# AdamClixby/Modulate

Hardware: NVIDIA B200
Metric: ark_dtb_decrypt_throughput (higher is better)
Workload: dtype u8

## Files before the change

### modulate_b200/csrc/cycle_kernels.cu

```cuda
#include "cycle_kernels.cuh"
#include "lcg.h"

#include <cstdlib>

namespace modk {

using modlcg::mulmod;
using modlcg::step_lazy;
using modlcg::low8_canonical;

#ifndef MODK_CANON_FMA_MASK
#define MODK_CANON_FMA_MASK 0x5
#endif
#ifndef MODK_MIN_CTAS
#define MODK_MIN_CTAS 10
#endif
#ifndef MODK_MIN_CTAS_INLINE
#define MODK_MIN_CTAS_INLINE 8
#endif
#ifndef MODK_MIN_CTAS_COAL
#define MODK_MIN_CTAS_COAL 10
#endif
#ifndef MODK_STAGE
#define MODK_STAGE 1
#endif
#ifndef MODK_EDGE_ROUNDS
#define MODK_EDGE_ROUNDS 1
#endif
#ifndef MODK_STAGE_SEQ
#define MODK_STAGE_SEQ 1
#endif
#ifndef MODK_GENERAL_FULL
#define MODK_GENERAL_FULL 1
#endif
#ifndef MODK_HOIST_POW
#define MODK_HOIST_POW 1
#endif
#ifndef MODK_REC_PREFETCH
#define MODK_REC_PREFETCH 2048
#endif

constexpr int kTw0Size = 1024;
constexpr int kTw1Size = (int)(((1ull << 32) / kTileBytes) / kTw0Size + 2);

__constant__ uint32_t c_tw0[kTw0Size];
__constant__ uint32_t c_tw1[kTw1Size];
__constant__ uint32_t c_ainv[16];
__device__ uint32_t g_chunk_pow2[kChunksPerTile];

__device__ __forceinline__ uint32_t jump_lazy(uint32_t st, uint32_t y2)
{
    const uint64_t p = (uint64_t)st * (uint64_t)y2;
    return (uint32_t)(p >> 32) + ((uint32_t)p >> 1);
}


__device__ __forceinline__ uint4 ldg128(uint64_t addr)
{
    uint4 r;
    asm volatile("ld.global.v4.u32 {%0, %1, %2, %3}, [%4];" : "=r"(r.x), "=r"(r.y), "=r"(r.z), "=r"(r.w) : "l"(addr));
    return r;
}

__device__ __forceinline__ void stg128(uint64_t addr, const uint4& v)
{
    asm volatile("st.global.v4.u32 [%0], {%1, %2, %3, %4};" ::"l"(addr), "r"(v.x), "r"(v.y), "r"(v.z), "r"(v.w));
}

#if MODK_STAGE

__device__ __forceinline__ uint32_t smem_u32(const void* p) { return (uint32_t)__cvta_generic_to_shared(p); }

__device__ __forceinline__ void mbar_init(uint32_t bar, uint32_t count)
{
    asm volatile("mbarrier.init.shared::cta.b64 [%0], %1;" ::"r"(bar), "r"(count));
    asm volatile("fence.mbarrier_init.release.cluster;" ::: "memory");
}

__device__ __forceinline__ void mbar_expect_tx(uint32_t bar, uint32_t bytes)
{
    asm volatile("mbarrier.arrive.expect_tx.shared::cta.b64 _, [%0], %1;" ::"r"(bar), "r"(bytes) : "memory");
}

__device__ __forceinline__ void mbar_wait(uint32_t bar, uint32_t parity)
{
    asm volatile(
        "{\n"
        ".reg .pred p;\n"
        "MODK_WAIT:\n"
        "mbarrier.try_wait.parity.shared::cta.b64 p, [%0], %1;\n"
        "@p bra MODK_DONE;\n"
        "bra MODK_WAIT;\n"
        "MODK_DONE:\n"
        "}\n" ::"r"(bar), "r"(parity) : "memory");
}

__device__ __forceinline__ void bulk_g2s(uint32_t dst_smem, uint64_t src_gmem, uint32_t bytes, uint32_t bar)
{
    asm volatile("cp.async.bulk.shared::cluster.global.mbarrier::complete_tx::bytes [%0], [%1], %2, [%3];" ::"r"(dst_smem),
                 "l"(src_gmem), "r"(bytes), "r"(bar)
                 : "memory");
}

__device__ __forceinline__ uint4 lds128(uint32_t addr)
{
    uint4 r;
    asm volatile("ld.shared.v4.u32 {%0, %1, %2, %3}, [%4];" : "=r"(r.x), "=r"(r.y), "=r"(r.z), "=r"(r.w) : "r"(addr));
    return r;
}
#endif


__device__ __forceinline__ uint32_t low8_canonical_fma(uint32_t s, uint32_t two)
{
    uint32_t r;
    asm("mad.hi.u32 %0, %1, %2, %1;" : "=r"(r) : "r"(s), "r"(two));
    return r;
}

// ... 231 lines not shown
        return;
    }
    constexpr bool kStaged = MODK_STAGE != 0;
#if MODK_STAGE
    if (threadIdx.x == 0) {
        const uint32_t bytes = 16u * (n_valid + (shift ? 1u : 0u));
        mbar_expect_tx(bar, bytes);
        bulk_g2s(stage, src_tile, bytes, bar);
    }
#endif
#if MODK_GENERAL_FULL
    if (geom == kFullGeom) {
        switch (shift ? (int)(shift >> 2) : -1) {
        case -1: process_tile<-1, U, kStaged, true>(src_tile, dst_tile, st, n_valid, head, tail, bs, idx0, pw, a.two, stage, bar); break;
        case 0: process_tile<0, U, kStaged, true>(src_tile, dst_tile, st, n_valid, head, tail, bs, idx0, pw, a.two, stage, bar); break;
        case 1: process_tile<1, U, kStaged, true>(src_tile, dst_tile, st, n_valid, head, tail, bs, idx0, pw, a.two, stage, bar); break;
        case 2: process_tile<2, U, kStaged, true>(src_tile, dst_tile, st, n_valid, head, tail, bs, idx0, pw, a.two, stage, bar); break;
        default: process_tile<3, U, kStaged, true>(src_tile, dst_tile, st, n_valid, head, tail, bs, idx0, pw, a.two, stage, bar); break;
        }
        return;
    }
#endif
    if (shift == 0u) {
        process_tile<-1, U, kStaged>(src_tile, dst_tile, st, n_valid, head, tail, bs, idx0, pw, a.two, stage, bar);
    } else {
        switch (shift >> 2) {
        case 0: process_tile<0, U, kStaged>(src_tile, dst_tile, st, n_valid, head, tail, bs, idx0, pw, a.two, stage, bar); break;
        case 1: process_tile<1, U, kStaged>(src_tile, dst_tile, st, n_valid, head, tail, bs, idx0, pw, a.two, stage, bar); break;
        case 2: process_tile<2, U, kStaged>(src_tile, dst_tile, st, n_valid, head, tail, bs, idx0, pw, a.two, stage, bar); break;
        default: process_tile<3, U, kStaged>(src_tile, dst_tile, st, n_valid, head, tail, bs, idx0, pw, a.two, stage, bar); break;
        }
    }
}

__device__ __forceinline__ uint32_t tile_start_state(uint32_t n0, uint32_t h0, uint32_t tin)
{
    const uint32_t st = mulmod(n0, c_ainv[h0]);
    return mulmod(st, mulmod(c_tw0[tin & (uint32_t)(kTw0Size - 1)], c_tw1[tin / (uint32_t)kTw0Size]));
}

__device__ __forceinline__ TileRec make_tile_rec(uint64_t src_off, uint64_t dst_off, uint32_t len, uint32_t n0,
                                                 uint32_t tin, uint32_t dst_align, uint32_t entry)
{
    const uint32_t h0 = (dst_align + (uint32_t)dst_off) & 15u;
    const uint64_t span = (uint64_t)h0 + len;
    const uint32_t nchunks = (uint32_t)((span + 15u) >> 4);
    const uint32_t c_begin = tin * (uint32_t)kChunksPerTile;
    const uint32_t n_valid = min((uint32_t)kChunksPerTile, nchunks - c_begin);
    const bool last = c_begin + n_valid == nchunks;
    TileRec r;
    r.src_rel = (int64_t)src_off - (int64_t)h0 + 16ll * (int64_t)c_begin;
    r.dst_rel = (int64_t)dst_off - (int64_t)h0 + 16ll * (int64_t)c_begin;
    r.state = tile_start_state(n0, h0, tin);
    r.geom = pack_geom(n_valid, tin == 0u ? h0 : 0u, last ? (((uint32_t)span - 1u) & 15u) + 1u : 16u);
    r.entry = entry;
    r.pad = 0u;
    return r;
}

#if MODK_STAGE
#define MODK_STAGE_SETUP                                                                          \
    uint32_t stage = 0u, bar = 0u;                                                                \
    if (kGeneral) {                                                                               \
        __shared__ __align__(128) uint8_t s_stage[kTileBytes + 16];                               \
        __shared__ __align__(8) uint64_t s_bar;                                                   \
        stage = smem_u32(s_stage);                                                                \
        bar = smem_u32(&s_bar);                                                                   \
        if (threadIdx.x == 0)                                                                     \
            mbar_init(bar, 1u);                                                                   \
        __syncthreads();                                                                          \
    }
#else
#define MODK_STAGE_SETUP const uint32_t stage = 0u, bar = 0u;
#endif

template <int U>
__device__ __forceinline__ void load_chunk_pows(uint32_t (&pw)[U], uint32_t idx0)
{
#pragma unroll
    for (int u = 0; u < U; ++u)
        pw[u] = __ldg(&g_chunk_pow2[idx0 + (uint32_t)u * (uint32_t)kThreadsPerCta]);
}

template <bool kGeneral>
__global__ void __launch_bounds__(kThreadsPerCta, kGeneral ? MODK_MIN_CTAS : MODK_MIN_CTAS_COAL)
cycle_batch_kernel(const BatchArgs a)
{
    MODK_STAGE_SETUP
    const uint4* p = reinterpret_cast<const uint4*>(a.tiles + blockIdx.x);
    uint32_t pw[kUnroll];
#if MODK_HOIST_POW
    load_chunk_pows<kUnroll>(pw, threadIdx.x);
#endif
    const uint4 lo = __ldg(p);
    const uint4 hi = __ldg(p + 1);
#if MODK_REC_PREFETCH
    if (threadIdx.x == 0 && a.n_tiles - blockIdx.x > (uint32_t)MODK_REC_PREFETCH) {
        const uint64_t ahead = (uint64_t)(a.tiles + blockIdx.x + MODK_REC_PREFETCH);
        if ((ahead & 127u) == 0u)
            asm volatile("prefetch.global.L2 [%0];" ::"l"(ahead));
    }
#endif
    const int64_t src_rel = (int64_t)((uint64_t)lo.x | ((uint64_t)lo.y << 32));
    const int64_t dst_rel = (int64_t)((uint64_t)lo.z | ((uint64_t)lo.w << 32));
#if !MODK_HOIST_POW
    load_chunk_pows<kUnroll>(pw, threadIdx.x);
#endif
    run_tile<kUnroll, kGeneral>(a, src_rel, dst_rel, hi.x, hi.y, threadIdx.x, pw, stage, bar);
}

template <bool kGeneral>
__global__ void __launch_bounds__(kThreadsPerCta, kGeneral ? MODK_MIN_CTAS_INLINE : MODK_MIN_CTAS_COAL)
cycle_inline_kernel(const BatchArgs a, const __grid_constant__ InlineDescs in)
{
    MODK_STAGE_SETUP
    uint32_t pw[kUnroll];
    load_chunk_pows<kUnroll>(pw, threadIdx.x);
    const uint32_t tile = blockIdx.x;
    const uint32_t e = tile / a.tiles_per_entry;
    const DevDesc& d = in.d[e];
    const TileRec r = make_tile_rec(d.src_off, d.dst_off, d.len, d.neg_state, tile - d.first_tile,
                                    (uint32_t)(uintptr_t)a.dst & 15u, e);
    run_tile<kUnroll, kGeneral>(a, r.src_rel, r.dst_rel, r.state, r.geom, threadIdx.x, pw, stage, bar);
}

__global__ void build_tiles_kernel(const DevDesc* __restrict__ descs, uint32_t n_descs, uint32_t dst_align,
                                   TileRec* __restrict__ tiles, uint32_t n_tiles)
{
    const uint32_t t = blockIdx.x * blockDim.x + threadIdx.x;
    if (t >= n_tiles)
        return;
    uint32_t lo = 0, hi = n_descs;
    while (hi - lo > 1) {
        const uint32_t mid = lo + ((hi - lo) >> 1);
        if (descs[mid].first_tile <= t)
            lo = mid;
        else
            hi = mid;
    }
    const DevDesc d = descs[lo];
    tiles[t] = make_tile_rec(d.src_off, d.dst_off, d.len, d.neg_state, t - d.first_tile, dst_align, lo);
}


cudaError_t upload_tables()
{
    static uint32_t h_tw0[kTw0Size], h_tw1[kTw1Size], h_ainv[16], h_chunk[kChunksPerTile];
    static const bool built = []() {
        for (int j = 0; j < kTw0Size; ++j)
            h_tw0[j] = modlcg::pow_a((uint64_t)kTileBytes * (uint64_t)j);
        for (int j = 0; j < kTw1Size; ++j)
            h_tw1[j] = modlcg::pow_a((uint64_t)kTileBytes * (uint64_t)kTw0Size * (uint64_t)j);
        for (int h = 0; h < 16; ++h)
            h_ainv[h] = modlcg::pow_a_inv((uint64_t)h);
        for (int j = 0; j < kChunksPerTile; ++j)
            h_chunk[j] = 2u * modlcg::pow_a(16ull * (uint64_t)j);
        return true;
    }();
    (void)built;
    cudaError_t err;
    if ((err = cudaMemcpyToSymbol(c_tw0, h_tw0, sizeof(h_tw0))) != cudaSuccess) return err;
    if ((err = cudaMemcpyToSymbol(c_tw1, h_tw1, sizeof(h_tw1))) != cudaSuccess) return err;
    if ((err = cudaMemcpyToSymbol(c_ainv, h_ainv, sizeof(h_ainv))) != cudaSuccess) return err;
    if ((err = cudaMemcpyToSymbol(g_chunk_pow2, h_chunk, sizeof(h_chunk))) != cudaSuccess) return err;
    return cudaSuccess;
}

constexpr uint32_t kMaxGrid = 0x7FFFFFFFu;

static bool coaligned(const BatchArgs& a)
{
    if (a.uniform_delta < 0 || getenv("MOD_FORCE_GENERAL") != nullptr)
        return false;
    return (((uintptr_t)a.src - (uintptr_t)a.dst + (uintptr_t)a.uniform_delta) & 15u) == 0u;
}

cudaError_t launch_batch(const BatchArgs& args, cudaStream_t stream)
{
    for (uint32_t t0 = 0; t0 < args.n_tiles;) {
        const uint32_t n = args.n_tiles - t0 < kMaxGrid ? args.n_tiles - t0 : kMaxGrid;
        BatchArgs a = args;
        a.tiles = args.tiles + t0;
        a.n_tiles = n;
        if (coaligned(args))
            cycle_batch_kernel<false><<<n, kThreadsPerCta, 0, stream>>>(a);
        else
            cycle_batch_kernel<true><<<n, kThreadsPerCta, 0, stream>>>(a);
        const cudaError_t err = cudaGetLastError();
        if (err != cudaSuccess)
            return err;
        t0 += n;
    }
    return cudaSuccess;
}

cudaError_t launch_batch_inline(const BatchArgs& args, const InlineDescs& descs, cudaStream_t stream)
{
    if (args.n_tiles == 0)
        return cudaSuccess;
    if (coaligned(args))
        cycle_inline_kernel<false><<<args.n_tiles, kThreadsPerCta, 0, stream>>>(args, descs);
    else
        cycle_inline_kernel<true><<<args.n_tiles, kThreadsPerCta, 0, stream>>>(args, descs);
    return cudaGetLastError();
}

cudaError_t launch_build_tiles(const DevDesc* descs, uint32_t n_descs, uint32_t dst_align, TileRec* tiles,
                               uint32_t n_tiles, cudaStream_t stream)
{
    if (n_tiles == 0)
        return cudaSuccess;
    const unsigned threads = 256;
    build_tiles_kernel<<<(n_tiles + threads - 1) / threads, threads, 0, stream>>>(descs, n_descs, dst_align,
                                                                                 tiles, n_tiles);
    return cudaGetLastError();
}

}
```

### modulate_b200/csrc/cycle_kernels.cuh

```cuda
#pragma once

#include <cuda_runtime.h>
#include <stdint.h>

namespace modk {

#ifndef MODK_THREADS
#define MODK_THREADS 128
#endif
#ifndef MODK_UNROLL
#define MODK_UNROLL 4
#endif
constexpr int kThreadsPerCta = MODK_THREADS;
constexpr int kUnroll = MODK_UNROLL;
constexpr int kChunksPerTile = kThreadsPerCta * kUnroll;
constexpr uint32_t kTileBytes = 16u * kChunksPerTile;
constexpr int kMaxInlineDescs = 64;
static_assert(kChunksPerTile <= 2048, "TileRec::geom holds the chunk count in 12 bits");

struct __align__(16) DevDesc {
    uint64_t src_off;
    uint64_t dst_off;
    uint32_t len;
    int32_t key;
    uint32_t first_tile;
    uint32_t neg_state;
};

struct __align__(16) TileRec {
    int64_t src_rel;
    int64_t dst_rel;
    uint32_t state;
    uint32_t geom;
    uint32_t entry;
    uint32_t pad;
};

__host__ __device__ inline uint32_t pack_geom(uint32_t n_valid, uint32_t head, uint32_t tail)
{
    return n_valid | (head << 12) | (tail << 16);
}

struct InlineDescs {
    DevDesc d[kMaxInlineDescs];
};

struct BatchArgs {
    const uint8_t* src;
    uint8_t* dst;
    const TileRec* tiles;
    uint32_t n_tiles;
    uint32_t tiles_per_entry;
    uint64_t src_lo16;
    uint64_t src_hi16;
    uint32_t two = 2;
    int32_t uniform_delta = -1;
};

__host__ __device__ inline uint32_t tiles_for_entry(uint32_t h0, uint32_t len)
{
    if (len == 0)
        return 0;
    const uint64_t chunks = ((uint64_t)h0 + len + 15u) >> 4;
    return (uint32_t)((chunks + (uint32_t)kChunksPerTile - 1) / (uint32_t)kChunksPerTile);
}

cudaError_t upload_tables();
cudaError_t launch_batch(const BatchArgs& args, cudaStream_t stream);
cudaError_t launch_batch_inline(const BatchArgs& args, const InlineDescs& descs, cudaStream_t stream);
cudaError_t launch_build_tiles(const DevDesc* descs, uint32_t n_descs, uint32_t dst_align, TileRec* tiles,
                               uint32_t n_tiles, cudaStream_t stream);

}
```

### modulate_b200/csrc/mod_abi.cu

```cuda
#include "../../include/modulate_b200.h"

#include <cuda_runtime.h>

#include <algorithm>
#include <atomic>
#include <chrono>
#include <cstdarg>
#include <cstdio>
#include <cstdlib>
#include <cstring>
#include <exception>
#include <mutex>
#include <new>
#include <string>
#include <thread>
#include <vector>

#include "batch_cut.h"
#include "cycle_kernels.cuh"
#include "lcg.h"

namespace {

#ifndef MOD_PIPE_SLOTS
// ... 232 lines not shown
        return fail(MOD_ERR_NOMEM, "cudaHostAlloc(%llu) failed: %s", (unsigned long long)need, cudaGetErrorString(e));
    }
    *have = need;
    return MOD_OK;
}

cudaError_t pool_alloc(DeviceCtx& c, uint64_t bytes, void** out, uint64_t* got)
{
    bytes = std::max<uint64_t>(256, (bytes + 255) & ~255ull);
    {
        std::lock_guard<std::mutex> lock(c.pool_mu);
        size_t best = c.pool.size();
        for (size_t i = 0; i < c.pool.size(); ++i)
            if (c.pool[i].bytes >= bytes && c.pool[i].bytes / 4 <= bytes && (best == c.pool.size() || c.pool[i].bytes < c.pool[best].bytes))
                best = i;
        if (best != c.pool.size()) {
            *out = c.pool[best].p;
            *got = c.pool[best].bytes;
            c.pool.erase(c.pool.begin() + (long)best);
            return cudaSuccess;
        }
    }
    *got = bytes;
    return cudaMalloc(out, bytes);
}

void pool_free(DeviceCtx& c, void* p, uint64_t bytes)
{
    if (!p)
        return;
    if (bytes <= kPoolMaxBlockBytes && c.ready.load(std::memory_order_acquire)) {
        std::lock_guard<std::mutex> lock(c.pool_mu);
        if (c.pool.size() >= kPoolBlocks) {
            size_t smallest = 0;
            for (size_t i = 1; i < c.pool.size(); ++i)
                if (c.pool[i].bytes < c.pool[smallest].bytes)
                    smallest = i;
            if (c.pool[smallest].bytes < bytes) {
                cudaFree(c.pool[smallest].p);
                c.pool[smallest] = DeviceCtx::Block{p, bytes};
                return;
            }
        } else {
            c.pool.push_back(DeviceCtx::Block{p, bytes});
            return;
        }
    }
    cudaFree(p);
}

int launch_contiguous(const uint8_t* d_src, uint8_t* d_dst, uint64_t len, int32_t key, cudaStream_t stream)
{
    if (len == 0)
        return MOD_OK;
    const uint32_t h0 = (uint32_t)((uintptr_t)d_dst & 15u);
    const uint64_t piece = kMaxPiece;
    const uint64_t src_lo16 = ((uint64_t)(uintptr_t)d_src + 15u) & ~15ull;
    const uint64_t src_hi16 = ((uint64_t)(uintptr_t)d_src + len) & ~15ull;
    const uint32_t tpe = modk::tiles_for_entry(h0, (uint32_t)piece);
    uint64_t done = 0;
    const uint32_t k0 = modlcg::key_residue(key);
    while (done < len) {
        modk::InlineDescs in;
        modk::BatchArgs args;
        uint32_t n = 0, tiles = 0;
        const uint64_t group_base = done;
        while (done < len && n < (uint32_t)modk::kMaxInlineDescs) {
            const uint64_t this_len = std::min(piece, len - done);
            modk::DevDesc& d = in.d[n];
            d.src_off = done - group_base;
            d.dst_off = done - group_base;
            d.len = (uint32_t)this_len;
            d.key = (int32_t)modlcg::mulmod(k0, modlcg::pow_a(done));
            d.first_tile = n * tpe;
            d.neg_state = modlcg::key_to_neg_state(d.key);
            tiles = n * tpe + modk::tiles_for_entry(h0, (uint32_t)this_len);
            done += this_len;
            ++n;
        }
        args.src = d_src + group_base;
        args.dst = d_dst + group_base;
        args.tiles = nullptr;
        args.n_tiles = tiles;
        args.tiles_per_entry = tpe;
        args.src_lo16 = src_lo16;
        args.src_hi16 = src_hi16;
        args.uniform_delta = 0;
        CUDA_TRY(modk::launch_batch_inline(args, in, stream));
        g_launches.fetch_add(1, std::memory_order_relaxed);
    }
    return MOD_OK;
}

int cycle_host(DeviceCtx& c, uint8_t* host, uint64_t len, int32_t key)
{
    std::lock_guard<std::mutex> lock(c.mu);
    uint64_t slice = env_u64("MOD_SLICE_BYTES", 16ull << 20);
    slice = std::max<uint64_t>(4096, slice & ~4095ull);
    if (len < slice * 2)
        slice = std::max<uint64_t>(4096, ((len / kPipeSlots) + 4095) & ~4095ull);
    const int slots = (int)std::min<uint64_t>(kPipeSlots, (len + slice - 1) / slice);
    for (int i = 0; i < slots; ++i) {
        const int rc = grow(&c.slice_buf[i], &c.slice_bytes[i], slice);
        if (rc != MOD_OK)
            return rc;
    }
    const uint32_t k0 = modlcg::key_residue(key);
    int rc = MOD_OK;
    cudaError_t e = cudaSuccess;
    uint64_t pos = 0;
    const uint64_t head = len >= 4 * slice ? ((kCopyAlign - ((uintptr_t)host & (kCopyAlign - 1))) & (kCopyAlign - 1)) : 0;
    for (uint64_t i = 0; pos < len && rc == MOD_OK && e == cudaSuccess; ++i) {
        const int slot = (int)(i % kPipeSlots);
        const uint64_t n = i == 0 && head ? head : std::min(slice, len - pos);
        cudaStream_t s = c.pipe_stream[slot];
        uint8_t* d = (uint8_t*)c.slice_buf[slot];
        e = cudaMemcpyAsync(d, host + pos, n, cudaMemcpyHostToDevice, s);
        if (e != cudaSuccess)
            break;
        rc = launch_contiguous(d, d, n, (int32_t)modlcg::mulmod(k0, modlcg::pow_a(pos)), s);
        if (rc != MOD_OK)
            break;
        e = cudaMemcpyAsync(host + pos, d, n, cudaMemcpyDeviceToHost, s);
        pos += n;
    }
    const cudaError_t ed = drain(c);
    if (rc != MOD_OK)
        return rc;
    if (e == cudaSuccess)
        e = ed;
    if (e != cudaSuccess)
        return fail(MOD_ERR_CUDA, "mod_cycle: %s", cudaGetErrorString(e));
    return MOD_OK;
}

int validate_descs(const char* who, const mod_desc* descs, uint64_t n, uint64_t src_bytes, uint64_t dst_bytes)
{
    for (uint64_t i = 0; i < n; ++i) {
        const mod_desc& d = descs[i];
        if (d.src_off > src_bytes || (uint64_t)d.len > src_bytes - d.src_off)
            return fail(MOD_ERR_ARG, "%s: descriptor %llu: source range [%llu, +%u) leaves the %llu-byte buffer", who,
                        (unsigned long long)i, (unsigned long long)d.src_off, d.len, (unsigned long long)src_bytes);
        if (d.dst_off > dst_bytes || (uint64_t)d.len > dst_bytes - d.dst_off)
            return fail(MOD_ERR_ARG, "%s: descriptor %llu: destination range [%llu, +%u) leaves the %llu-byte buffer", who,
                        (unsigned long long)i, (unsigned long long)d.dst_off, d.len, (unsigned long long)dst_bytes);
    }
    return MOD_OK;
}

int32_t uniform_delta_of(const mod_desc* descs, uint64_t n)
{
    int32_t delta = -1;
    for (uint64_t i = 0; i < n; ++i) {
        if (!descs[i].len)
            continue;
        const int32_t d = (int32_t)((descs[i].src_off - descs[i].dst_off) & 15u);
        if (delta < 0)
            delta = d;
        else if (delta != d)
            return -1;
    }
    return delta;
}

int expand_descs(const mod_desc* descs, uint64_t n, uint32_t dst_align, modk::DevDesc* out, uint64_t* tiles_out,
                 uint64_t* payload_out)
{
    uint64_t tiles = 0, payload = 0;
    for (uint64_t i = 0; i < n; ++i) {
        const mod_desc& d = descs[i];
        modk::DevDesc& o = out[i];
// ... 153 lines not shown
                    gaps.push_back(gap);
                }
                runs.back().second = b1;
            } else {
                runs.emplace_back(b0, b1);
            }
            prev_rank = rank[idx];
        }
    };
    std::vector<std::pair<uint64_t, uint64_t>> runs;
    bool holes = false;
    for (const Group& g : groups) {
        merged_runs(g, runs, false);
        if (runs.size() > 64) {
            holes = true;
            break;
        }
    }
    if (holes)
        whole();

    const bool split_downloads = env_u64("MOD_SPLIT_DOWNLOADS", 1) != 0;
    const int slots = (int)std::min<size_t>(kPipeSlots, groups.size());
    {
        uint64_t s_need = 0, d_need = 0;
        for (const Group& g : groups) {
            s_need = std::max<uint64_t>(s_need, (g.s_lo & 15u) + (g.s_hi - g.s_lo) + 3 * kCopyAlign);
            d_need = std::max<uint64_t>(d_need, g.d_hi - (g.d_lo & ~15ull) + kCopyAlign);
        }
        for (int k = 0; k < slots; ++k) {
            if ((rc = grow(&c.slot_src[k], &c.slot_src_bytes[k], s_need)) != MOD_OK)
                return rc;
            if ((rc = grow(&c.slot_dst[k], &c.slot_dst_bytes[k], d_need)) != MOD_OK)
                return rc;
        }
    }

    cudaError_t e = cudaMemcpyAsync(c.ws_descs, c.h_descs, n * sizeof(modk::DevDesc), cudaMemcpyHostToDevice, c.pipe_stream[0]);
    if (e == cudaSuccess) {
        e = modk::launch_build_tiles((const modk::DevDesc*)c.ws_descs, (uint32_t)n, 0, (modk::TileRec*)c.ws_tiles,
                                     (uint32_t)plan_tiles, c.pipe_stream[0]);
        g_launches.fetch_add(1, std::memory_order_relaxed);
    }
    if (e == cudaSuccess)
        e = cudaEventRecord(c.plan_ready, c.pipe_stream[0]);
    const modk::TileRec* d_tiles = (const modk::TileRec*)c.ws_tiles;
    const int32_t uniform_delta = uniform_delta_of(descs, n);
    const double t_plan = now_ms();

    const uint64_t fail_group = env_u64("MOD_TEST_FAIL_GROUP", UINT64_MAX);
    for (size_t gi = 0; gi < groups.size() && e == cudaSuccess; ++gi) {
        if (gi == fail_group) {
            e = cudaErrorUnknown;
            break;
        }
        const Group& g = groups[gi];
        const int k = (int)(gi % (size_t)slots);
        cudaStream_t s = c.pipe_stream[k];
        const uint64_t d_lo16 = g.d_lo & ~15ull;
        uint64_t up_lo = g.s_lo, up_hi = g.s_hi;
        uint8_t* win_src = (uint8_t*)c.slot_src[k] + (g.s_lo & 15u);
        uint8_t* win_dst = (uint8_t*)c.slot_dst[k];
        if (align_copies) {
            up_lo -= std::min<uint64_t>(g.s_lo, (uintptr_t)(src + g.s_lo) & (kCopyAlign - 1));
            up_hi = std::min<uint64_t>(src_bytes, g.s_hi + ((kCopyAlign - ((uintptr_t)(src + g.s_hi) & (kCopyAlign - 1))) & (kCopyAlign - 1)));
            win_src = (uint8_t*)c.slot_src[k] + ((uintptr_t)(src + up_lo) & (kCopyAlign - 1)) + (g.s_lo - up_lo);
            win_dst = (uint8_t*)c.slot_dst[k] + ((uintptr_t)(dst + d_lo16) & (kCopyAlign - 1));
        }
        e = cudaMemcpyAsync(win_src - (g.s_lo - up_lo), src + up_lo, up_hi - up_lo, cudaMemcpyHostToDevice, s);
        if (e == cudaSuccess && holes)
            e = cudaMemcpyAsync(win_dst, dst + d_lo16, g.d_hi - d_lo16, cudaMemcpyHostToDevice, s);
        if (e != cudaSuccess)
            break;
        if (!holes)
            merged_runs(g, runs, true);
        if (gi > 0 && gi < (size_t)slots) {
            e = cudaStreamWaitEvent(s, c.plan_ready, 0);
            if (e != cudaSuccess)
                break;
        }
        modk::BatchArgs args;
        args.src = win_src - g.s_lo;
        args.dst = win_dst - d_lo16;
        args.tiles = d_tiles + g.t0;
        args.n_tiles = g.t1 - g.t0;
        args.tiles_per_entry = 0;
        args.src_lo16 = ((uint64_t)(uintptr_t)(win_src - (g.s_lo - up_lo)) + 15u) & ~15ull;
        args.src_hi16 = ((uint64_t)(uintptr_t)(win_src + (up_hi - g.s_lo))) & ~15ull;
        args.uniform_delta = uniform_delta;
        e = modk::launch_batch(args, s);
        g_launches.fetch_add(1, std::memory_order_relaxed);
        if (e != cudaSuccess)
            break;
        if (holes) {
            e = cudaMemcpyAsync(dst + d_lo16, win_dst, g.d_hi - d_lo16, cudaMemcpyDeviceToHost, s);
        } else {
            for (const auto& r : runs) {
                uint64_t cut[4] = {r.first, r.first, r.second, r.second};
                if (align_copies && split_downloads && r.second - r.first >= (64u << 10)) {
                    cut[1] = r.first + ((kCopyAlign - ((uintptr_t)(dst + r.first) & (kCopyAlign - 1))) & (kCopyAlign - 1));
                    cut[2] = r.second - ((uintptr_t)(dst + r.second) & (kCopyAlign - 1));
                }
                for (int q = 0; q < 3 && e == cudaSuccess; ++q)
                    if (cut[q + 1] > cut[q])
                        e = cudaMemcpyAsync(dst + cut[q], win_dst + (cut[q] - d_lo16), cut[q + 1] - cut[q],
                                            cudaMemcpyDeviceToHost, s);
                if (e != cudaSuccess)
                    break;
            }
        }
    }
    const double t_enq = now_ms();
    const cudaError_t ed = drain(c);
    if (e == cudaSuccess)
        e = ed;
    if (e == cudaSuccess)
        for (const Gap& gap : gaps)
            std::memcpy(dst + gap.off, gap.bytes, gap.len);
    if (trace)
        fprintf(stderr, "[mod] cycle_batch dev %d: plan %.2f ms, enqueue %zu groups %.2f ms, drain %.2f ms\n", c.device,
                t_plan - t_begin, groups.size(), t_enq - t_plan, now_ms() - t_enq);
    if (e != cudaSuccess)
        return fail(MOD_ERR_CUDA, "mod_cycle_batch: %s", cudaGetErrorString(e));
    return MOD_OK;
}


int selected_devices(uint64_t dev_mask, std::vector<int>& out)
{
    int count = 0;
    CUDA_TRY(cudaGetDeviceCount(&count));
    if (count <= 0)
        return fail(MOD_ERR_CUDA, "no CUDA device visible: this library has no CPU fallback");
    for (int d = 0; d < count && d < kMaxDevices; ++d)
        if (dev_mask == 0 || ((dev_mask >> d) & 1ull))
            out.push_back(d);
    if (out.empty())
        return fail(MOD_ERR_ARG, "dev_mask 0x%llx selects none of the %d visible devices", (unsigned long long)dev_mask, count);
    return MOD_OK;
}

template <class F>
int for_each_device(uint64_t dev_mask, F fn)
{
    std::vector<int> devs;
    int rc = selected_devices(dev_mask, devs);
    if (rc != MOD_OK)
        return rc;
    const int world = (int)devs.size();
    std::vector<int> rcs((size_t)world, MOD_OK);
    std::vector<std::string> errs((size_t)world);
    auto body = [&](int r) {
        try {
            DeviceCtx* c = nullptr;
            int my = acquire(devs[(size_t)r], &c);
            if (my == MOD_OK)
                my = fn(r, world, *c);
            rcs[(size_t)r] = my;
        } catch (const std::bad_alloc&) {
            rcs[(size_t)r] = fail(MOD_ERR_NOMEM, "out of host memory");
        } catch (...) {
            rcs[(size_t)r] = fail(MOD_ERR_ARG, "unexpected exception");
        }
        if (rcs[(size_t)r] != MOD_OK)
            errs[(size_t)r] = tl_error;
    };
    if (world == 1) {
        int prev = 0;
        CUDA_TRY(cudaGetDevice(&prev));
        body(0);
        cudaSetDevice(prev);
    } else {
        std::vector<std::thread> threads;
        threads.reserve((size_t)world);
        for (int r = 0; r < world; ++r)
            threads.emplace_back(body, r);
        for (std::thread& t : threads)
            t.join();
    }
    for (int r = 0; r < world; ++r) {
        if (rcs[(size_t)r] != MOD_OK) {
            tl_error = "device " + std::to_string(devs[(size_t)r]) + ": " + errs[(size_t)r];
            return rcs[(size_t)r];
        }
    }
    return MOD_OK;
}

}

struct mod_plan {
    int device = -1;
    uint64_t n = 0;
    uint64_t src_bytes = 0;
    uint64_t dst_bytes = 0;
    uint32_t dst_align = 0;
    uint64_t payload = 0;
    uint32_t n_tiles = 0;
    int32_t uniform_delta = -1;
    modk::TileRec* d_tiles = nullptr;
    uint64_t d_tiles_bytes = 0;
    std::vector<mod_desc> descs;
    std::vector<uint32_t> first_tile;
};

extern "C" {

int mod_abi_version(void) { return MOD_ABI_VERSION; }

const char* mod_last_error(void) { return tl_error.c_str(); }

uint64_t mod_launch_count(void) { return g_launches.load(std::memory_order_relaxed); }

int mod_device_count(void)
{
    int count = 0;
    cudaError_t e = cudaGetDeviceCount(&count);
    if (e != cudaSuccess) {
        cudaGetLastError();
        return fail(MOD_ERR_CUDA, "cudaGetDeviceCount: %s", cudaGetErrorString(e));
    }
    return count;
}

int mod_init(int device)
{
    DeviceCtx* c = nullptr;
    return acquire(device, &c);
}

int mod_current_device(void)
{
    int cur = -1;
    CUDA_TRY(cudaGetDevice(&cur));
    return cur;
}

int mod_is_device_pointer(const void* p)
{
    int dev = -1;
    return pointer_device(p, &dev) ? 1 : 0;
}

void mod_shutdown(void)
{
    std::lock_guard<std::mutex> init_lock(g_init_mu);
    int prev = -1;
    cudaGetDevice(&prev);
    for (int d = 0; d < kMaxDevices; ++d) {
        DeviceCtx& c = g_dev[d];
        if (!c.ready.load(std::memory_order_acquire))
            continue;
        std::lock_guard<std::mutex> lock(c.mu);
        if (cudaSetDevice(d) != cudaSuccess) {
            cudaGetLastError();
            continue;
        }
        cudaDeviceSynchronize();
        release_ctx(c);
    }
    if (prev >= 0)
        cudaSetDevice(prev);
}


void* mod_host_alloc(uint64_t bytes)
{
    void* p = nullptr;
    cudaError_t e = cudaHostAlloc(&p, bytes ? bytes : 1, cudaHostAllocPortable);
    if (e != cudaSuccess) {
        cudaGetLastError();
        fail(MOD_ERR_NOMEM, "cudaHostAlloc(%llu): %s", (unsigned long long)bytes, cudaGetErrorString(e));
        return nullptr;
    }
    return p;
}

int mod_host_free(void* p)
{
    if (!p)
        return MOD_OK;
    CUDA_TRY(cudaFreeHost(p));
// ... 102 lines not shown
        return MOD_OK;
    }
    DeviceCtx* c = nullptr;
    int rc = acquire(-1, &c);
    if (rc != MOD_OK)
        return rc;
    return cycle_host(*c, (uint8_t*)data, len, key);
    MOD_ABI_END("mod_cycle")
}

int mod_cycle_sharded(void* data, uint64_t len, int32_t key, uint64_t dev_mask)
{
    MOD_ABI_BEGIN
    if (len == 0)
        return MOD_OK;
    if (!data)
        return fail(MOD_ERR_ARG, "mod_cycle_sharded: null pointer");
    int ptr_dev = -1;
    if (pointer_device(data, &ptr_dev))
        return fail(MOD_ERR_ARG, "mod_cycle_sharded: `data` must be a host buffer (a device buffer lives on one GPU: use mod_cycle)");
    uint8_t* host = (uint8_t*)data;
    return for_each_device(dev_mask, [=](int rank, int world, DeviceCtx& c) -> int {
        uint64_t b = 0, e = 0;
        int rc = mod_shard_range(len, rank, world, &b, &e);
        if (rc != MOD_OK || e <= b)
            return rc;
        return cycle_host(c, host + b, e - b, mod_key_jump(key, b));
    });
    MOD_ABI_END("mod_cycle_sharded")
}


int mod_plan_create(const mod_desc* descs, uint64_t n, uint64_t src_bytes, uint64_t dst_bytes,
                    uint32_t dst_align, mod_plan** out)
{
    MOD_ABI_BEGIN
    if (!out)
        return fail(MOD_ERR_ARG, "mod_plan_create: out is null");
    *out = nullptr;
    if (n && !descs)
        return fail(MOD_ERR_ARG, "mod_plan_create: descs is null");
    if (n >= 0xFFFFFFFFull)
        return fail(MOD_ERR_ARG, "mod_plan_create: too many descriptors (%llu)", (unsigned long long)n);
    if (dst_align > 15)
        return fail(MOD_ERR_ARG, "mod_plan_create: dst_align must be < 16");
    DeviceCtx* c = nullptr;
    int rc = acquire(-1, &c);
    if (rc != MOD_OK)
        return rc;
    if ((rc = validate_descs("mod_plan_create", descs, n, src_bytes, dst_bytes)) != MOD_OK)
        return rc;

    std::vector<modk::DevDesc> host(n);
    uint64_t tiles = 0, payload = 0;
    if ((rc = expand_descs(descs, n, dst_align, host.data(), &tiles, &payload)) != MOD_OK)
        return rc;

    mod_plan* p = new mod_plan();
    p->device = c->device;
    p->n = n;
    p->src_bytes = src_bytes;
    p->dst_bytes = dst_bytes;
    p->dst_align = dst_align;
    p->payload = payload;
    p->n_tiles = (uint32_t)tiles;
    p->uniform_delta = uniform_delta_of(descs, n);
    modk::DevDesc* d_descs = nullptr;
    uint64_t d_descs_bytes = 0;
    auto cleanup = [&]() {
        pool_free(*c, d_descs, d_descs_bytes);
        pool_free(*c, p->d_tiles, p->d_tiles_bytes);
        delete p;
    };
    try {
        p->descs.assign(descs, descs + n);
        p->first_tile.resize(n + 1);
        for (uint64_t i = 0; i < n; ++i)
            p->first_tile[i] = host[i].first_tile;
        p->first_tile[n] = (uint32_t)tiles;
    } catch (...) {
        cleanup();
        throw;
    }
    if (n && tiles) {
        cudaError_t e = pool_alloc(*c, n * sizeof(modk::DevDesc), (void**)&d_descs, &d_descs_bytes);
        if (e == cudaSuccess)
            e = pool_alloc(*c, tiles * sizeof(modk::TileRec), (void**)&p->d_tiles, &p->d_tiles_bytes);
        if (e != cudaSuccess) {
            cudaGetLastError();
            cleanup();
            return fail(MOD_ERR_NOMEM, "mod_plan_create: cudaMalloc failed: %s", cudaGetErrorString(e));
        }
        e = cudaMemcpy(d_descs, host.data(), n * sizeof(modk::DevDesc), cudaMemcpyHostToDevice);
        if (e == cudaSuccess) {
            e = modk::launch_build_tiles(d_descs, (uint32_t)n, dst_align, p->d_tiles, p->n_tiles, nullptr);
            g_launches.fetch_add(1, std::memory_order_relaxed);
        }
        if (e == cudaSuccess)
            e = cudaStreamSynchronize(nullptr);
        if (e != cudaSuccess) {
            cleanup();
            return fail(MOD_ERR_CUDA, "mod_plan_create: %s", cudaGetErrorString(e));
        }
        pool_free(*c, d_descs, d_descs_bytes);
        d_descs = nullptr;
    }
    *out = p;
    return MOD_OK;
    MOD_ABI_END("mod_plan_create")
}

int mod_plan_destroy(mod_plan* plan)
{
    if (!plan)
        return MOD_OK;
    if (plan->d_tiles) {
        DeviceGuard guard;
        guard.enter(plan->device);
        cudaDeviceSynchronize();
        if (plan->device >= 0 && plan->device < kMaxDevices)
            pool_free(g_dev[plan->device], plan->d_tiles, plan->d_tiles_bytes);
        else
            cudaFree(plan->d_tiles);
    }
    delete plan;
    return MOD_OK;
}

uint64_t mod_plan_payload_bytes(const mod_plan* plan) { return plan ? plan->payload : 0; }
uint64_t mod_plan_num_tiles(const mod_plan* plan) { return plan ? plan->n_tiles : 0; }

int mod_plan_tile_range(const mod_plan* plan, uint64_t entry_begin, uint64_t entry_end, uint64_t* tile_begin,
                        uint64_t* tile_end)
{
    if (!plan || !tile_begin || !tile_end)
        return fail(MOD_ERR_ARG, "mod_plan_tile_range: null argument");
    if (entry_begin > entry_end || entry_end > plan->n)
        return fail(MOD_ERR_ARG, "mod_plan_tile_range: entries [%llu, %llu) outside the plan's %llu",
                    (unsigned long long)entry_begin, (unsigned long long)entry_end, (unsigned long long)plan->n);
    *tile_begin = plan->first_tile[entry_begin];
    *tile_end = plan->first_tile[entry_end];
    return MOD_OK;
}

static int plan_check_device(const mod_plan* plan, const char* who)
{
    int cur = -1;
    CUDA_TRY(cudaGetDevice(&cur));
    if (cur != plan->device)
        return fail(MOD_ERR_ARG, "%s: the plan lives on device %d but the calling thread is bound to device %d", who,
                    plan->device, cur);
    return MOD_OK;
}

int mod_plan_run(const mod_plan* plan, const void* d_src, void* d_dst, void* stream)
{
    if (!plan)
        return fail(MOD_ERR_ARG, "mod_plan_run: null plan");
    if (plan->n_tiles == 0)
        return MOD_OK;
    if (!d_src || !d_dst)
        return fail(MOD_ERR_ARG, "mod_plan_run: null buffer");
    if (((uintptr_t)d_dst & 15u) != plan->dst_align)
        return fail(MOD_ERR_ALIGN, "mod_plan_run: dst & 15 is %u but the plan was built for %u",
                    (unsigned)((uintptr_t)d_dst & 15u), plan->dst_align);
    int rc = plan_check_device(plan, "mod_plan_run");
    if (rc != MOD_OK)
        return rc;
    modk::BatchArgs args;
    args.src = (const uint8_t*)d_src;
    args.dst = (uint8_t*)d_dst;
    args.tiles = plan->d_tiles;
    args.n_tiles = plan->n_tiles;
    args.tiles_per_entry = 0;
    args.src_lo16 = ((uint64_t)(uintptr_t)d_src + 15u) & ~15ull;
    args.src_hi16 = ((uint64_t)(uintptr_t)d_src + plan->src_bytes) & ~15ull;
    args.uniform_delta = plan->uniform_delta;
    CUDA_TRY(modk::launch_batch(args, (cudaStream_t)stream));
    g_launches.fetch_add(1, std::memory_order_relaxed);
    return MOD_OK;
}

int mod_plan_run_window(const mod_plan* plan, uint64_t tile_begin, uint64_t tile_end, const void* d_src_win,
                        uint64_t src_win_off, uint64_t src_win_bytes, void* d_dst_win, uint64_t dst_win_off,
                        uint64_t dst_win_bytes, void* stream)
{
    if (!plan)
        return fail(MOD_ERR_ARG, "mod_plan_run_window: null plan");
    if (tile_begin > tile_end || tile_end > plan->n_tiles)
        return fail(MOD_ERR_ARG, "mod_plan_run_window: tiles [%llu, %llu) outside the plan's %u",
                    (unsigned long long)tile_begin, (unsigned long long)tile_end, plan->n_tiles);
    if (tile_begin == tile_end)
        return MOD_OK;
    if (!d_src_win || !d_dst_win)
        return fail(MOD_ERR_ARG, "mod_plan_run_window: null buffer");
    if ((((uintptr_t)d_dst_win - dst_win_off) & 15u) != plan->dst_align)
        return fail(MOD_ERR_ALIGN, "mod_plan_run_window: (d_dst_win - dst_win_off) & 15 is %u but the plan was built for %u",
                    (unsigned)(((uintptr_t)d_dst_win - dst_win_off) & 15u), plan->dst_align);
    int rc = plan_check_device(plan, "mod_plan_run_window");
    if (rc != MOD_OK)
        return rc;
    const uint32_t* ft = plan->first_tile.data();
    uint64_t e = (uint64_t)(std::upper_bound(ft, ft + plan->n + 1, (uint32_t)tile_begin) - ft) - 1;
    for (; e < plan->n && ft[e] < tile_end; ++e) {
        const mod_desc& d = plan->descs[e];
        if (ft[e + 1] == ft[e])
            continue;
        const uint32_t h0 = (uint32_t)((plan->dst_align + d.dst_off) & 15u);
        const uint64_t ta = std::max<uint64_t>(tile_begin, ft[e]) - ft[e], tb = std::min<uint64_t>(tile_end, ft[e + 1]) - ft[e];
        const uint64_t b0 = ta == 0 ? 0 : ta * modk::kTileBytes - h0;
        const uint64_t b1 = std::min<uint64_t>(d.len, tb * modk::kTileBytes - h0);
        if (d.src_off + b0 < src_win_off || d.src_off + b1 > src_win_off + src_win_bytes)
            return fail(MOD_ERR_ARG, "mod_plan_run_window: entry %llu reads outside the source window", (unsigned long long)e);
        if (d.dst_off + b0 < dst_win_off || d.dst_off + b1 > dst_win_off + dst_win_bytes)
            return fail(MOD_ERR_ARG, "mod_plan_run_window: entry %llu writes outside the destination window", (unsigned long long)e);
    }
    modk::BatchArgs args;
    args.src = (const uint8_t*)d_src_win - src_win_off;
    args.dst = (uint8_t*)d_dst_win - dst_win_off;
    args.tiles = plan->d_tiles + tile_begin;
    args.n_tiles = (uint32_t)(tile_end - tile_begin);
    args.tiles_per_entry = 0;
    args.src_lo16 = ((uint64_t)(uintptr_t)d_src_win + 15u) & ~15ull;
    args.src_hi16 = ((uint64_t)(uintptr_t)d_src_win + src_win_bytes) & ~15ull;
    args.uniform_delta = plan->uniform_delta;
    CUDA_TRY(modk::launch_batch(args, (cudaStream_t)stream));
    g_launches.fetch_add(1, std::memory_order_relaxed);
    return MOD_OK;
}

int mod_cycle_batch(const mod_desc* descs, uint64_t n, const void* src, uint64_t src_bytes, void* dst,
                    uint64_t dst_bytes)
{
    MOD_ABI_BEGIN
    if (n == 0)
        return MOD_OK;
    if (!descs)
        return fail(MOD_ERR_ARG, "mod_cycle_batch: descs is null");
    if (!src || !dst)
        return fail(MOD_ERR_ARG, "mod_cycle_batch: null buffer");
    int src_dev = -1, dst_dev = -1;
    const bool src_is_dev = pointer_device(src, &src_dev), dst_is_dev = pointer_device(dst, &dst_dev);
    if (src_is_dev != dst_is_dev || (src_is_dev && src_dev != dst_dev))
        return fail(MOD_ERR_ARG, "mod_cycle_batch: src and dst must both be host pointers or both live on one device");

    if (src_is_dev) {
        DeviceGuard guard;
        int rc = guard.enter(src_dev);
        if (rc != MOD_OK)
            return rc;
        mod_plan* plan = nullptr;
        rc = mod_plan_create(descs, n, src_bytes, dst_bytes, (uint32_t)((uintptr_t)dst & 15u), &plan);
        if (rc != MOD_OK)
            return rc;
        rc = mod_plan_run(plan, src, dst, nullptr);
        cudaError_t e = cudaStreamSynchronize(nullptr);
        mod_plan_destroy(plan);
        if (rc != MOD_OK)
            return rc;
        CUDA_TRY(e);
        return MOD_OK;
    }
    DeviceCtx* c = nullptr;
    int rc = acquire(-1, &c);
    if (rc != MOD_OK)
        return rc;
    return batch_host(*c, descs, n, (const uint8_t*)src, src_bytes, (uint8_t*)dst, dst_bytes);
    MOD_ABI_END("mod_cycle_batch")
}

int mod_cycle_batch_sharded(const mod_desc* descs, uint64_t n, const void* src, uint64_t src_bytes, void* dst,
                            uint64_t dst_bytes, uint64_t dev_mask)
{
    MOD_ABI_BEGIN
    if (n == 0)
        return MOD_OK;
    if (!descs)
        return fail(MOD_ERR_ARG, "mod_cycle_batch_sharded: descs is null");
    if (!src || !dst)
        return fail(MOD_ERR_ARG, "mod_cycle_batch_sharded: null buffer");
    int dev = -1;
    if (pointer_device(src, &dev) || pointer_device(dst, &dev))
        return fail(MOD_ERR_ARG, "mod_cycle_batch_sharded: src and dst must be host buffers");
    int rc = validate_descs("mod_cycle_batch_sharded", descs, n, src_bytes, dst_bytes);
    if (rc != MOD_OK)
        return rc;
    return for_each_device(dev_mask, [=](int rank, int world, DeviceCtx& c) -> int {
        if (world == 1)
            return batch_host(c, descs, n, (const uint8_t*)src, src_bytes, (uint8_t*)dst, dst_bytes);
        const int64_t count = mod_shard_descs(descs, n, rank, world, nullptr, 0);
        if (count < 0)
            return (int)count;
        if (count == 0)
            return MOD_OK;
        std::vector<mod_desc> shard((size_t)count);
        const int64_t got = mod_shard_descs(descs, n, rank, world, shard.data(), (uint64_t)count);
        if (got < 0)
            return (int)got;
        return batch_host(c, shard.data(), (uint64_t)got, (const uint8_t*)src, src_bytes, (uint8_t*)dst, dst_bytes);
    });
    MOD_ABI_END("mod_cycle_batch_sharded")
}


int mod_shard_range(uint64_t total, int rank, int world, uint64_t* begin, uint64_t* end)
{
    if (world <= 0 || rank < 0 || rank >= world || !begin || !end)
        return fail(MOD_ERR_ARG, "mod_shard_range: bad rank %d / world %d", rank, world);
    const uint64_t share = ((total / (uint64_t)world) + 15u) & ~15ull;
// ... 70 lines not shown
```

Measured before the change: 3463.

## Enable programmatic dependent launch and inline descriptors for small plans

Merges the batch and inline kernels into one templated kernel launched with cudaLaunchKernelEx and programmatic stream serialization. Each CTA does its prologue (power loads, descriptor binary search) before griddepcontrol.wait, so it can overlap the tail of the previous kernel. Plans with up to 64 descriptors now pass their descriptors as a grid constant instead of reading tile records from global memory. The inline path now does a per-CTA binary search instead of a division, and the change also adds optional timeline instrumentation.

```diff
diff --git a/modulate_b200/csrc/cycle_kernels.cu b/modulate_b200/csrc/cycle_kernels.cu
--- a/modulate_b200/csrc/cycle_kernels.cu
+++ b/modulate_b200/csrc/cycle_kernels.cu
@@ -33,8 +33,8 @@
 #ifndef MODK_GENERAL_FULL
 #define MODK_GENERAL_FULL 1
 #endif
-#ifndef MODK_HOIST_POW
-#define MODK_HOIST_POW 1
+#ifndef MODK_PDL
+#define MODK_PDL 1
 #endif
 #ifndef MODK_REC_PREFETCH
 #define MODK_REC_PREFETCH 2048
@@ -432,46 +432,84 @@
         pw[u] = __ldg(&g_chunk_pow2[idx0 + (uint32_t)u * (uint32_t)kThreadsPerCta]);
 }
 
-template <bool kGeneral>
-__global__ void __launch_bounds__(kThreadsPerCta, kGeneral ? MODK_MIN_CTAS : MODK_MIN_CTAS_COAL)
-cycle_batch_kernel(const BatchArgs a)
-{
-    MODK_STAGE_SETUP
-    const uint4* p = reinterpret_cast<const uint4*>(a.tiles + blockIdx.x);
-    uint32_t pw[kUnroll];
-#if MODK_HOIST_POW
-    load_chunk_pows<kUnroll>(pw, threadIdx.x);
-#endif
-    const uint4 lo = __ldg(p);
-    const uint4 hi = __ldg(p + 1);
-#if MODK_REC_PREFETCH
-    if (threadIdx.x == 0 && a.n_tiles - blockIdx.x > (uint32_t)MODK_REC_PREFETCH) {
-        const uint64_t ahead = (uint64_t)(a.tiles + blockIdx.x + MODK_REC_PREFETCH);
-        if ((ahead & 127u) == 0u)
-            asm volatile("prefetch.global.L2 [%0];" ::"l"(ahead));
-    }
-#endif
-    const int64_t src_rel = (int64_t)((uint64_t)lo.x | ((uint64_t)lo.y << 32));
-    const int64_t dst_rel = (int64_t)((uint64_t)lo.z | ((uint64_t)lo.w << 32));
-#if !MODK_HOIST_POW
-    load_chunk_pows<kUnroll>(pw, threadIdx.x);
-#endif
-    run_tile<kUnroll, kGeneral>(a, src_rel, dst_rel, hi.x, hi.y, threadIdx.x, pw, stage, bar);
-}
-
-template <bool kGeneral>
-__global__ void __launch_bounds__(kThreadsPerCta, kGeneral ? MODK_MIN_CTAS_INLINE : MODK_MIN_CTAS_COAL)
-cycle_inline_kernel(const BatchArgs a, const __grid_constant__ InlineDescs in)
-{
+__device__ __forceinline__ void grid_dep_wait() { asm volatile("griddepcontrol.wait;" ::: "memory"); }
+__device__ __forceinline__ void grid_dep_launch_dependents() { asm volatile("griddepcontrol.launch_dependents;" ::: "memory"); }
+
+#ifdef MODK_TIMELINE
+__device__ __forceinline__ uint64_t globaltimer_after(uint32_t dep)
+{
+    uint64_t t = 0;
+    if (dep != 0xFFFFFFFFu)
+        asm volatile("mov.u64 %0, %%globaltimer;" : "=l"(t)::"memory");
+    return t;
+}
+#define MODK_TL(k, dep)                                                       \
+    if (threadIdx.x == 0)                                                     \
+        a.timeline[8ull * blockIdx.x + (k)] = globaltimer_after(dep);
+#else
+#define MODK_TL(k, dep)
+#endif
+
+template <bool kGeneral, bool kInline>
+__global__ void __launch_bounds__(kThreadsPerCta, !kGeneral ? MODK_MIN_CTAS_COAL : kInline ? MODK_MIN_CTAS_INLINE : MODK_MIN_CTAS)
+cycle_batch_kernel(const BatchArgs a, const __grid_constant__ InlineDescs in)
+{
+    MODK_TL(0, 0u)
     MODK_STAGE_SETUP
     uint32_t pw[kUnroll];
     load_chunk_pows<kUnroll>(pw, threadIdx.x);
-    const uint32_t tile = blockIdx.x;
-    const uint32_t e = tile / a.tiles_per_entry;
-    const DevDesc& d = in.d[e];
-    const TileRec r = make_tile_rec(d.src_off, d.dst_off, d.len, d.neg_state, tile - d.first_tile,
-                                    (uint32_t)(uintptr_t)a.dst & 15u, e);
-    run_tile<kUnroll, kGeneral>(a, r.src_rel, r.dst_rel, r.state, r.geom, threadIdx.x, pw, stage, bar);
+    const uint32_t tile = a.tile0 + blockIdx.x;
+    int64_t src_rel, dst_rel;
+    uint32_t st, geom;
+    if (kInline) {
+        uint32_t lo = 0, hi = a.n_descs;
+        while (hi - lo > 1) {
+            const uint32_t mid = lo + ((hi - lo) >> 1);
+            if (in.d[mid].first_tile <= tile)
+                lo = mid;
+            else
+                hi = mid;
+        }
+        const DevDesc& d = in.d[lo];
+        const TileRec r = make_tile_rec(d.src_off, d.dst_off, d.len, d.neg_state, tile - d.first_tile,
+                                        (uint32_t)(uintptr_t)a.dst & 15u, lo);
+        src_rel = r.src_rel;
+        dst_rel = r.dst_rel;
+        st = r.state;
+        geom = r.geom;
+        MODK_TL(1, st)
+        grid_dep_wait();
+        MODK_TL(2, 0u)
+    } else {
+        grid_dep_wait();
+        MODK_TL(2, 0u)
+        const uint4* p = reinterpret_cast<const uint4*>(a.tiles + tile);
+        const uint4 lo = __ldg(p);
+        const uint4 hi = __ldg(p + 1);
+#if MODK_REC_PREFETCH
+        if (threadIdx.x == 0 && a.n_tiles - blockIdx.x > (uint32_t)MODK_REC_PREFETCH) {
+            const uint64_t ahead = (uint64_t)(a.tiles + tile + MODK_REC_PREFETCH);
+            if ((ahead & 127u) == 0u)
+                asm volatile("prefetch.global.L2 [%0];" ::"l"(ahead));
+        }
+#endif
+        src_rel = (int64_t)((uint64_t)lo.x | ((uint64_t)lo.y << 32));
+        dst_rel = (int64_t)((uint64_t)lo.z | ((uint64_t)lo.w << 32));
+        st = hi.x;
+        geom = hi.y;
+        MODK_TL(1, st)
+    }
+    grid_dep_launch_dependents();
+    run_tile<kUnroll, kGeneral>(a, src_rel, dst_rel, st, geom, threadIdx.x, pw, stage, bar);
+#ifdef MODK_TIMELINE
+    __syncthreads();
+    MODK_TL(3, 0u)
+    if (threadIdx.x == 0) {
+        uint32_t sm;
+        asm volatile("mov.u32 %0, %%smid;" : "=r"(sm));
+        a.timeline[8ull * blockIdx.x + 4] = sm;
+    }
+#endif
 }
 
 __global__ void build_tiles_kernel(const DevDesc* __restrict__ descs, uint32_t n_descs, uint32_t dst_align,
@@ -525,34 +563,43 @@
     return (((uintptr_t)a.src - (uintptr_t)a.dst + (uintptr_t)a.uniform_delta) & 15u) == 0u;
 }
 
-cudaError_t launch_batch(const BatchArgs& args, cudaStream_t stream)
-{
+template <bool kGeneral, bool kInline>
+static cudaError_t launch_one(const BatchArgs& a, const InlineDescs& in, cudaStream_t stream)
+{
+    cudaLaunchAttribute attr[1];
+    attr[0].id = cudaLaunchAttributeProgrammaticStreamSerialization;
+    attr[0].val.programmaticStreamSerializationAllowed = MODK_PDL;
+    cudaLaunchConfig_t cfg = {};
+    cfg.gridDim = dim3(a.n_tiles);
+    cfg.blockDim = dim3(kThreadsPerCta);
+    cfg.stream = stream;
+    cfg.attrs = attr;
+    cfg.numAttrs = 1;
+    return cudaLaunchKernelEx(&cfg, cycle_batch_kernel<kGeneral, kInline>, a, in);
+}
+
+cudaError_t launch_batch(const BatchArgs& args, const InlineDescs* descs, cudaStream_t stream)
+{
+    static const InlineDescs kNoDescs = {};
+    const bool co = coaligned(args);
     for (uint32_t t0 = 0; t0 < args.n_tiles;) {
         const uint32_t n = args.n_tiles - t0 < kMaxGrid ? args.n_tiles - t0 : kMaxGrid;
         BatchArgs a = args;
-        a.tiles = args.tiles + t0;
+        a.tile0 = args.tile0 + t0;
         a.n_tiles = n;
-        if (coaligned(args))
-            cycle_batch_kernel<false><<<n, kThreadsPerCta, 0, stream>>>(a);
+#ifdef MODK_TIMELINE
+        a.timeline = args.timeline + 8ull * t0;
+#endif
+        cudaError_t err;
+        if (descs)
+            err = co ? launch_one<false, true>(a, *descs, stream) : launch_one<true, true>(a, *descs, stream);
         else
-            cycle_batch_kernel<true><<<n, kThreadsPerCta, 0, stream>>>(a);
-        const cudaError_t err = cudaGetLastError();
+            err = co ? launch_one<false, false>(a, kNoDescs, stream) : launch_one<true, false>(a, kNoDescs, stream);
         if (err != cudaSuccess)
             return err;
         t0 += n;
     }
     return cudaSuccess;
-}
-
-cudaError_t launch_batch_inline(const BatchArgs& args, const InlineDescs& descs, cudaStream_t stream)
-{
-    if (args.n_tiles == 0)
-        return cudaSuccess;
-    if (coaligned(args))
-        cycle_inline_kernel<false><<<args.n_tiles, kThreadsPerCta, 0, stream>>>(args, descs);
-    else
-        cycle_inline_kernel<true><<<args.n_tiles, kThreadsPerCta, 0, stream>>>(args, descs);
-    return cudaGetLastError();
 }
 
 cudaError_t launch_build_tiles(const DevDesc* descs, uint32_t n_descs, uint32_t dst_align, TileRec* tiles,
diff --git a/modulate_b200/csrc/cycle_kernels.cuh b/modulate_b200/csrc/cycle_kernels.cuh
--- a/modulate_b200/csrc/cycle_kernels.cuh
+++ b/modulate_b200/csrc/cycle_kernels.cuh
@@ -49,12 +49,16 @@
     const uint8_t* src;
     uint8_t* dst;
     const TileRec* tiles;
+    uint32_t tile0 = 0;
     uint32_t n_tiles;
-    uint32_t tiles_per_entry;
+    uint32_t n_descs = 0;
     uint64_t src_lo16;
     uint64_t src_hi16;
     uint32_t two = 2;
     int32_t uniform_delta = -1;
+#ifdef MODK_TIMELINE
+    uint64_t* timeline = nullptr;
+#endif
 };
 
 __host__ __device__ inline uint32_t tiles_for_entry(uint32_t h0, uint32_t len)
@@ -66,8 +70,7 @@
 }
 
 cudaError_t upload_tables();
-cudaError_t launch_batch(const BatchArgs& args, cudaStream_t stream);
-cudaError_t launch_batch_inline(const BatchArgs& args, const InlineDescs& descs, cudaStream_t stream);
+cudaError_t launch_batch(const BatchArgs& args, const InlineDescs* descs, cudaStream_t stream);
 cudaError_t launch_build_tiles(const DevDesc* descs, uint32_t n_descs, uint32_t dst_align, TileRec* tiles,
                                uint32_t n_tiles, cudaStream_t stream);
 
diff --git a/modulate_b200/csrc/mod_abi.cu b/modulate_b200/csrc/mod_abi.cu
--- a/modulate_b200/csrc/mod_abi.cu
+++ b/modulate_b200/csrc/mod_abi.cu
@@ -338,11 +338,11 @@
         args.dst = d_dst + group_base;
         args.tiles = nullptr;
         args.n_tiles = tiles;
-        args.tiles_per_entry = tpe;
+        args.n_descs = n;
         args.src_lo16 = src_lo16;
         args.src_hi16 = src_hi16;
         args.uniform_delta = 0;
-        CUDA_TRY(modk::launch_batch_inline(args, in, stream));
+        CUDA_TRY(modk::launch_batch(args, &in, stream));
         g_launches.fetch_add(1, std::memory_order_relaxed);
     }
     return MOD_OK;
@@ -662,13 +662,13 @@
         modk::BatchArgs args;
         args.src = win_src - g.s_lo;
         args.dst = win_dst - d_lo16;
-        args.tiles = d_tiles + g.t0;
+        args.tiles = d_tiles;
+        args.tile0 = g.t0;
         args.n_tiles = g.t1 - g.t0;
-        args.tiles_per_entry = 0;
         args.src_lo16 = ((uint64_t)(uintptr_t)(win_src - (g.s_lo - up_lo)) + 15u) & ~15ull;
         args.src_hi16 = ((uint64_t)(uintptr_t)(win_src + (up_hi - g.s_lo))) & ~15ull;
         args.uniform_delta = uniform_delta;
-        e = modk::launch_batch(args, s);
+        e = modk::launch_batch(args, nullptr, s);
         g_launches.fetch_add(1, std::memory_order_relaxed);
         if (e != cudaSuccess)
             break;
@@ -778,6 +778,8 @@
     uint64_t payload = 0;
     uint32_t n_tiles = 0;
     int32_t uniform_delta = -1;
+    bool inline_descs = false;
+    modk::InlineDescs in;
     modk::TileRec* d_tiles = nullptr;
     uint64_t d_tiles_bytes = 0;
     std::vector<mod_desc> descs;
@@ -1046,7 +1048,10 @@
         cleanup();
         throw;
     }
-    if (n && tiles) {
+    if (n <= (uint64_t)modk::kMaxInlineDescs) {
+        p->inline_descs = true;
+        std::copy(host.begin(), host.end(), p->in.d);
+    } else if (tiles) {
         cudaError_t e = pool_alloc(*c, n * sizeof(modk::DevDesc), (void**)&d_descs, &d_descs_bytes);
         if (e == cudaSuccess)
             e = pool_alloc(*c, tiles * sizeof(modk::TileRec), (void**)&p->d_tiles, &p->d_tiles_bytes);
@@ -1136,11 +1141,11 @@
     args.dst = (uint8_t*)d_dst;
     args.tiles = plan->d_tiles;
     args.n_tiles = plan->n_tiles;
-    args.tiles_per_entry = 0;
+    args.n_descs = (uint32_t)plan->n;
     args.src_lo16 = ((uint64_t)(uintptr_t)d_src + 15u) & ~15ull;
     args.src_hi16 = ((uint64_t)(uintptr_t)d_src + plan->src_bytes) & ~15ull;
     args.uniform_delta = plan->uniform_delta;
-    CUDA_TRY(modk::launch_batch(args, (cudaStream_t)stream));
+    CUDA_TRY(modk::launch_batch(args, plan->inline_descs ? &plan->in : nullptr, (cudaStream_t)stream));
     g_launches.fetch_add(1, std::memory_order_relaxed);
     return MOD_OK;
 }
@@ -1182,13 +1187,14 @@
     modk::BatchArgs args;
     args.src = (const uint8_t*)d_src_win - src_win_off;
     args.dst = (uint8_t*)d_dst_win - dst_win_off;
-    args.tiles = plan->d_tiles + tile_begin;
+    args.tiles = plan->d_tiles;
+    args.tile0 = (uint32_t)tile_begin;
     args.n_tiles = (uint32_t)(tile_end - tile_begin);
-    args.tiles_per_entry = 0;
+    args.n_descs = (uint32_t)plan->n;
     args.src_lo16 = ((uint64_t)(uintptr_t)d_src_win + 15u) & ~15ull;
     args.src_hi16 = ((uint64_t)(uintptr_t)d_src_win + src_win_bytes) & ~15ull;
     args.uniform_delta = plan->uniform_delta;
-    CUDA_TRY(modk::launch_batch(args, (cudaStream_t)stream));
+    CUDA_TRY(modk::launch_batch(args, plan->inline_descs ? &plan->in : nullptr, (cudaStream_t)stream));
     g_launches.fetch_add(1, std::memory_order_relaxed);
     return MOD_OK;
 }
```

After: 3471 (median of 6 runs). Within noise of the previous version (+0.2%).
